# vlazzarini/opencl_fft

Hardware: AMD Instinct MI355X
Metric: Gsamples/s for batched 1D FFT (N=65536, float32) + achieved HBM GB/s vs peak (higher is better)
Workload: dtype f32; 1 GPU; c2c N=65536 x 4096 batches per GPU, float32, in place, device-resident (BASELINE configs[1]); direction=steps alternate forward/inverse plans, kernel=k_fft_res16, global_batch=4096, settle_launches=70, effective_warmup_launches=75, library=opencl_fft_amd/libclfft_amd.so

## Files before the change

include/clfft_amd.h:

```cpp
#ifndef CLFFT_AMD_H
#define CLFFT_AMD_H

#include <stddef.h>

#ifdef __cplusplus
extern "C" {
#endif

#define CLFA_API __attribute__((visibility("default")))

#define CLFA_SUCCESS 0
#define CLFA_DEVICE_NOT_FOUND (-1)
#define CLFA_DEVICE_NOT_AVAILABLE (-2)
#define CLFA_MEM_OBJECT_ALLOCATION_FAILURE (-4)
#define CLFA_OUT_OF_RESOURCES (-5)
#define CLFA_OUT_OF_HOST_MEMORY (-6)
#define CLFA_INVALID_VALUE (-30)
#define CLFA_INVALID_DEVICE (-33)
#define CLFA_INVALID_COMMAND_QUEUE (-36)
#define CLFA_INVALID_MEM_OBJECT (-38)
#define CLFA_INVALID_KERNEL_ARGS (-52)
#define CLFA_INVALID_OPERATION (-59)
#define CLFA_INVALID_BUFFER_SIZE (-61)

// ... 12 lines not shown
CLFA_API int clfa_bitrev_table(int n, int *out);
CLFA_API int clfa_twiddle_table(int n, int forward, float *out);
CLFA_API int clfa_r2c_twiddle_table(int m, int forward, float *out);

CLFA_API int clfa_cfft_create(clfa_fft **plan, int device, int n, int forward);
CLFA_API int clfa_rfft_create(clfa_fft **plan, int device, int size, int forward);
CLFA_API void clfa_fft_destroy(clfa_fft *plan);
CLFA_API int clfa_fft_get_error(const clfa_fft *plan);
CLFA_API const char *clfa_fft_get_log(const clfa_fft *plan);
CLFA_API int clfa_cfft_transform(clfa_fft *plan, float *c, long batch);
CLFA_API int clfa_rfft_transform(clfa_fft *plan, float *c, float *r, long batch);
CLFA_API int clfa_fft_host_alloc(clfa_fft *plan, size_t bytes, void **ptr);
CLFA_API int clfa_fft_host_free(clfa_fft *plan, void *ptr);
CLFA_API int clfa_fft_exec_dev(clfa_fft *plan, void *data, long batch, void *stream);
CLFA_API int clfa_fft_exec_dev_oop(clfa_fft *plan, const void *src, void *dst, long batch, void *stream);
CLFA_API int clfa_fft_device_buffers(clfa_fft *plan, void **data1, void **data2, void **commands);
CLFA_API int clfa_fft_device_tables(clfa_fft *plan, void **w, void **b);
CLFA_API int clfa_copy_to_device(void *stream, void *dst, const void *src, size_t bytes, int blocking);
CLFA_API int clfa_copy_from_device(void *stream, void *dst, const void *src, size_t bytes, int blocking);
CLFA_API int clfa_stream_synchronize(void *stream);
CLFA_API int clfa_fft_run_buffers(clfa_fft *plan);
CLFA_API size_t clfa_fft_workspace_bytes(const clfa_fft *plan);
CLFA_API const char *clfa_fft_kernel_name(const clfa_fft *plan);

CLFA_API int clfa_bandwidth_probe(int device, int what, size_t bytes, int launches, double *tb_per_s);

CLFA_API int clfa_reorder_dev(int device, void *out, const void *in, int n, long batch, void *stream);

CLFA_API int clfa_pconv_create(clfa_pconv **pc, int device, int cvs, int pts, int channels);
CLFA_API void clfa_pconv_destroy(clfa_pconv *pc);
CLFA_API int clfa_pconv_get_error(const clfa_pconv *pc);
CLFA_API int clfa_pconv_nparts(const clfa_pconv *pc);
CLFA_API int clfa_pconv_wp(const clfa_pconv *pc);
CLFA_API int clfa_pconv_wp2(const clfa_pconv *pc);
CLFA_API int clfa_pconv_push_ir(clfa_pconv *pc, const float *ir);
CLFA_API int clfa_pconv_push_ir_dev(clfa_pconv *pc, const void *ir, long channel_stride, void *stream);
CLFA_API int clfa_pconv_convolution(clfa_pconv *pc, float *out, const float *in);
CLFA_API int clfa_pconv_convolution_tv(clfa_pconv *pc, float *out, const float *in1, const float *in2);
CLFA_API int clfa_pconv_process_dev(clfa_pconv *pc, void *out, const void *in1, const void *in2, void *stream);
CLFA_API size_t clfa_pconv_state_bytes(const clfa_pconv *pc);
CLFA_API const char *clfa_pconv_kernel_name(const clfa_pconv *pc);
CLFA_API int clfa_pconv_process_blocks_dev(clfa_pconv *pc, void *out, long out_stride, const void *in1, const void *in2,
                                           long in_stride, long nblocks, void *stream);
CLFA_API int clfa_pconv_convolution_blocks(clfa_pconv *pc, float *out, const float *in1, const float *in2, long nblocks);
CLFA_API size_t clfa_pconv_blocks_workspace_bytes(const clfa_pconv *pc);
CLFA_API const char *clfa_pconv_blocks_kernel_name(const clfa_pconv *pc);
// ... 157 lines not shown
```

opencl_fft_amd/_lib.py:

```python
import ctypes as C
import os

_HERE = os.path.dirname(os.path.abspath(__file__))
LIB_PATH = os.environ.get("CLFA_LIB_PATH") or os.path.join(_HERE, "libclfft_amd.so")
if os.environ.get("CLFA_LIB_PATH"):
    import sys
    print("opencl_fft_amd: CLFA_LIB_PATH is set, loading %s instead of the in-tree library" % LIB_PATH, file=sys.stderr)

_vp, _fp, _ip = C.c_void_p, C.POINTER(C.c_float), C.POINTER(C.c_int)
SYMBOLS = [
    ("clfa_device_count", C.c_int, [_ip]),
    ("clfa_device_name", C.c_int, [C.c_int, C.c_char_p, C.c_size_t]),
    ("clfa_error_string", C.c_char_p, [C.c_int]),
    ("clfa_version", C.c_char_p, []),
    ("clfa_bitrev_table", C.c_int, [C.c_int, _ip]),
    ("clfa_twiddle_table", C.c_int, [C.c_int, C.c_int, _fp]),
    ("clfa_r2c_twiddle_table", C.c_int, [C.c_int, C.c_int, _fp]),
    ("clfa_cfft_create", C.c_int, [C.POINTER(_vp), C.c_int, C.c_int, C.c_int]),
    ("clfa_rfft_create", C.c_int, [C.POINTER(_vp), C.c_int, C.c_int, C.c_int]),
    ("clfa_fft_destroy", None, [_vp]),
    ("clfa_fft_get_error", C.c_int, [_vp]),
    ("clfa_fft_get_log", C.c_char_p, [_vp]),
    ("clfa_cfft_transform", C.c_int, [_vp, _vp, C.c_long]),
    ("clfa_rfft_transform", C.c_int, [_vp, _vp, _vp, C.c_long]),
    ("clfa_fft_host_alloc", C.c_int, [_vp, C.c_size_t, C.POINTER(_vp)]),
    ("clfa_fft_host_free", C.c_int, [_vp, _vp]),
    ("clfa_fft_exec_dev", C.c_int, [_vp, _vp, C.c_long, _vp]),
    ("clfa_fft_exec_dev_oop", C.c_int, [_vp, _vp, _vp, C.c_long, _vp]),
    ("clfa_fft_device_buffers", C.c_int, [_vp, C.POINTER(_vp), C.POINTER(_vp), C.POINTER(_vp)]),
    ("clfa_fft_run_buffers", C.c_int, [_vp]),
    ("clfa_fft_device_tables", C.c_int, [_vp, C.POINTER(_vp), C.POINTER(_vp)]),
    ("clfa_copy_to_device", C.c_int, [_vp, _vp, _vp, C.c_size_t, C.c_int]),
    ("clfa_copy_from_device", C.c_int, [_vp, _vp, _vp, C.c_size_t, C.c_int]),
    ("clfa_stream_synchronize", C.c_int, [_vp]),
    ("clfa_fft_workspace_bytes", C.c_size_t, [_vp]),
    ("clfa_fft_kernel_name", C.c_char_p, [_vp]),
    ("clfa_reorder_dev", C.c_int, [C.c_int, _vp, _vp, C.c_int, C.c_long, _vp]),
    ("clfa_pconv_create", C.c_int, [C.POINTER(_vp), C.c_int, C.c_int, C.c_int, C.c_int]),
    ("clfa_pconv_destroy", None, [_vp]),
    ("clfa_pconv_get_error", C.c_int, [_vp]),
    ("clfa_pconv_nparts", C.c_int, [_vp]),
    ("clfa_pconv_wp", C.c_int, [_vp]),
    ("clfa_pconv_wp2", C.c_int, [_vp]),
    ("clfa_pconv_push_ir", C.c_int, [_vp, _vp]),
    ("clfa_pconv_push_ir_dev", C.c_int, [_vp, _vp, C.c_long, _vp]),
    ("clfa_bandwidth_probe", C.c_int, [C.c_int, C.c_int, C.c_size_t, C.c_int, C.POINTER(C.c_double)]),
    ("clfa_pconv_convolution", C.c_int, [_vp, _vp, _vp]),
    ("clfa_pconv_convolution_tv", C.c_int, [_vp, _vp, _vp, _vp]),
    ("clfa_pconv_process_dev", C.c_int, [_vp, _vp, _vp, _vp, _vp]),
    ("clfa_pconv_state_bytes", C.c_size_t, [_vp]),
    ("clfa_pconv_kernel_name", C.c_char_p, [_vp]),
    ("clfa_pconv_process_blocks_dev", C.c_int, [_vp, _vp, C.c_long, _vp, _vp, C.c_long, C.c_long, _vp]),
    ("clfa_pconv_convolution_blocks", C.c_int, [_vp, _vp, _vp, _vp, C.c_long]),
    ("clfa_pconv_blocks_workspace_bytes", C.c_size_t, [_vp]),
    ("clfa_pconv_blocks_kernel_name", C.c_char_p, [_vp]),
    ("clfa_pconv_matrix_create", C.c_int, [C.POINTER(_vp), C.c_int, C.c_int, C.c_int, C.c_int, C.c_int]),
    ("clfa_pconv_matrix_destroy", None, [_vp]),
    ("clfa_pconv_matrix_get_error", C.c_int, [_vp]),
    ("clfa_pconv_matrix_get_log", C.c_char_p, [_vp]),
# ... 144 lines not shown
```

opencl_fft_amd/csrc/clfft_amd.cpp:

```cpp
#include <utility>

#include "host.hpp"

using namespace clfa;


struct clfa_fft {
  DeviceInfo di;
  FftShape sh;
  int size = 0;
  int err = 0;
  char log[2048];
  hipStream_t stream = nullptr;
  DevBuf half, w2, four, scratch, stage, res16;
  DevBuf own1, own2;
  DevBuf own_w, own_b;
  bool own_tables_ready = false;
  struct Pinned {
    char *h, *d;
    size_t bytes;
  };
  std::vector<Pinned> pinned;
  clfa_fft *own_cplx = nullptr;
  StreamOrder order;
  HostBuf zstage;
  FftTables tabs;
  BigGeom big{};
  DevBuf bigtabs, scratch2;
  clfa_fft *blue_f = nullptr, *blue_i = nullptr;
  DevBuf blue_w, blue_b, blue_work;
};

extern "C" {


const char *clfa_version(void) { return "clfft_amd 0.1 (gfx950)"; }

int clfa_device_count(int *count) {
  if (!count) return CLFA_INVALID_VALUE;
  int c = 0;
  hipError_t e = hipGetDeviceCount(&c);
  if (e != hipSuccess || c <= 0) {
    (void)hipGetLastError();
    *count = 0;
    return CLFA_DEVICE_NOT_FOUND;
  }
  *count = c;
  return CLFA_SUCCESS;
}

int clfa_device_name(int device, char *buf, size_t len) {
// ... 151 lines not shown
    fill_big_tables(h, n, 1 << p->big.logn1);
    if ((e = upload(p->bigtabs, h.data(), sizeof(cpx) * h.size()))) return e;
    const long mb = env_long("CLFA_BIG_CHUNK_MB", 0, 1L << 31);
    const size_t per = sizeof(cpx) * (size_t)n;
    if ((e = p->scratch.ensure(per * chunk_items(per, (size_t)(mb ? mb : 256) << 20)))) return e;
  }
  const unsigned needs = fft_needs(rows);
  auto put = [&](DevBuf &b, const cpx *&tab) {
    const int err = upload(b, h.data(), sizeof(cpx) * h.size());
    tab = (const cpx *)b.p;
    return err;
  };
  if (needs & (kNeedHalf | kNeedHalf2x)) {
    if (needs & kNeedHalf2x) fill_lane_tables(h, rows.logn - 1, rows.logn == 14);
    else if (kLdsTwoLevel(rows.logn)) fill_lane_tables(h, rows.logn, false);
    else fill_twiddle(h, rows.n / 2, rows.n, 1, -1.f);
    if ((e = put(p->half, p->tabs.half))) return e;
  }
  if (needs & kNeedFour) fill_fourstep_tables(h, rows.logn);
  if ((needs & kNeedFour) && (e = put(p->four, p->tabs.four))) return e;
  if (needs & kNeedRes16) fill_res16_tables(h);
  if ((needs & kNeedRes16) && (e = put(p->res16, p->tabs.res16))) return e;
  DevBuf &ws = rows.logn == p->sh.logn ? p->scratch : p->scratch2;
  return needs & kNeedFourWs ? ws.ensure((size_t)fourstep_grid(p->di) * rows.n * sizeof(cpx)) : CLFA_SUCCESS;
}

int clfa_cfft_create(clfa_fft **plan, int device, int n, int forward) {
  return create_object(plan, [&](clfa_fft *p) { return fft_setup(p, device, n, false, n, forward != 0); });
}

int clfa_rfft_create(clfa_fft **plan, int device, int size, int forward) {
  return create_object(plan, [&](clfa_fft *p) {
    if (size < 4 || (size & 1)) {
      snprintf(p->log, sizeof(p->log), "real size must be even, 4..%d (got %d)", 2 << kBigMaxLog, size);
      return CLFA_INVALID_VALUE;
    }
    return fft_setup(p, device, size / 2, true, size, forward != 0);
  });
}

void clfa_fft_destroy(clfa_fft *p) {
  destroy_object(p, [](clfa_fft *q) {
    for (auto &r : q->pinned) (void)hipHostFree(r.h);
    q->pinned.clear();
    if (q->own_cplx) clfa_fft_destroy(q->own_cplx);
    if (q->blue_f) clfa_fft_destroy(q->blue_f);
    if (q->blue_i) clfa_fft_destroy(q->blue_i);
// ... 27 lines not shown
  });
}

static int fft_exec(clfa_fft *p, cpx *d, long off, long batch, hipStream_t s) {
  const FftShape &sh = p->sh;
  const bool fwd = sh.fwd, scale = sh.fwd;
  const FftRoute route = fft_route(sh, batch);
  const bool apart = sh.real && route_pack_apart(route);
  cpx *o = d + off, *scratch = (cpx *)p->scratch.p;
  if (apart && !fwd) {
    HIP_TRY(launch_c2r_unpack(d, p->tabs.w2, sh.n, batch, s, off));
    d = o;
  }
  switch (route) {
    case FftRoute::Lds: HIP_TRY(launch_fft_lds(sh.logn, fwd, fft_mode(sh), scale, d, p->tabs, batch, p->di, s, off)); break;
    case FftRoute::Cfft2x13: HIP_TRY(launch_cfft_2x13(fwd, scale, d, p->tabs, batch, p->di, s, off)); break;
    case FftRoute::Rfft2x13: HIP_TRY(launch_rfft_2x13(fwd, d, p->tabs, batch, p->di, s, off)); break;
    case FftRoute::Rfft2x14: HIP_TRY(launch_rfft_lds15(fwd, d, p->tabs, batch, p->di, s, off)); break;
    case FftRoute::RealRes16:
      if (fwd) HIP_TRY(launch_rfft_res16(d, o, scratch, p->tabs.res16, p->tabs.w2, batch, p->di, s));
      else HIP_TRY(launch_crfft_res16(d, o, scratch, p->tabs.res16, p->tabs.w2, batch, p->di, s));
      break;
    case FftRoute::FourStepSpread:
    case FftRoute::FourStep:
    case FftRoute::Res16: HIP_TRY(launch_fft_4step(sh.logn, fwd, scale, d, scratch, p->tabs, batch, p->di, s, o - d)); break;
    case FftRoute::Big: {
      const int e = for_chunks(batch, (long)(p->scratch.bytes / (sizeof(cpx) * (size_t)sh.n)), [&](long b0, long nb) -> int {
        HIP_TRY(launch_fft_big(p->big, fwd, scale, d + b0 * (long)sh.n, o + b0 * (long)sh.n, scratch, (cpx *)p->scratch2.p,
                               (const cpx *)p->bigtabs.p, p->tabs, nb, p->di, s));
        return CLFA_SUCCESS;
      });
      if (e) return e;
      break;
    }
    case FftRoute::BlueLds:
      HIP_TRY(launch_blue_lds(sh.blue_m, d, o, (const cpx *)p->blue_w.p, (const cpx *)p->blue_b.p, p->blue_f->tabs.half, sh.n,
                              (scale ? 1.0f / (float)sh.n : 1.0f) / (float)sh.blue_m, batch, p->di, s));
      break;
    case FftRoute::Bluestein:
      if (int e = blue_exec(p, d, o, batch, s)) return e;
      break;
  }
  if (apart && fwd) HIP_TRY(launch_r2c_pack(o, p->tabs.w2, sh.n, batch, s));
  return CLFA_SUCCESS;
}

int clfa_fft_exec_dev(clfa_fft *p, void *data, long batch, void *stream) {
  if (int e = obj_error(p)) return e;
  if (!data || batch < 0) return CLFA_INVALID_VALUE;
  if (batch == 0) return CLFA_SUCCESS;
  ENTER_DEVICE(p->di.device);
  hipStream_t s = (hipStream_t)stream;
  HIP_TRY(p->order.use(s));
  return fft_exec(p, (cpx *)data, 0, batch, s);
}

int clfa_fft_exec_dev_oop(clfa_fft *p, const void *src, void *dst, long batch, void *stream) {
  if (int e = obj_error(p)) return e;
  if (!src || !dst || batch < 0) return CLFA_INVALID_VALUE;
  if (src == dst) return clfa_fft_exec_dev(p, dst, batch, stream);
  if (batch == 0) return CLFA_SUCCESS;
  const size_t bytes = sizeof(cpx) * (size_t)p->sh.n * (size_t)batch;
  const char *a = (const char *)src, *b = (const char *)dst;
  if (spans_overlap(a, bytes, b, bytes)) return CLFA_INVALID_VALUE;
  if ((b - a) % (long)sizeof(cpx)) return CLFA_INVALID_VALUE;
  ENTER_DEVICE(p->di.device);
  hipStream_t s = (hipStream_t)stream;
  HIP_TRY(p->order.use(s));
  return fft_exec(p, (cpx *)const_cast<void *>(src), (long)((b - a) / (long)sizeof(cpx)), batch, s);
}

int clfa_fft_device_buffers(clfa_fft *p, void **data1, void **data2, void **commands) {
  if (int e = obj_error(p)) return e;
  ENTER_DEVICE(p->di.device);
  const size_t bytes = sizeof(cpx) * (size_t)p->sh.n;
  int e = p->own1.ensure(bytes);
  if (!e) e = p->own2.ensure(bytes);
  if (e) return e;
  if (data1) *data1 = p->own1.p;
  if (data2) *data2 = p->own2.p;
  if (commands) *commands = (void *)p->stream;
  return CLFA_SUCCESS;
}

int clfa_fft_device_tables(clfa_fft *p, void **w, void **b) {
  if (int e = obj_error(p)) return e;
  if (p->sh.blue_m || p->sh.logn < 1 || p->sh.logn > kMaxLog) return CLFA_INVALID_OPERATION;
  ENTER_DEVICE(p->di.device);
  const int n = p->sh.n;
  if (!p->own_tables_ready) {
    std::vector<cpx> tw;
    fill_twiddle(tw, n, n, 1, p->sh.fwd ? -1.f : 1.f);
// ... 145 lines not shown
```

opencl_fft_amd/csrc/fft_device.hpp:

```cpp
#pragma once
#include <type_traits>

#if defined(__HIPCC__)
#include <hip/hip_runtime.h>
#define CLFA_HD __host__ __device__ __forceinline__
#else
#define CLFA_HD inline
#endif

namespace clfa {

CLFA_HD long xcd_first(unsigned i, unsigned grid) {
  if (grid & 7) return i;
  return (long)(i & 7) * (grid >> 3) + (i >> 3);
}


#if defined(__clang__)
typedef float cpx __attribute__((ext_vector_type(2)));
#define CLFA_VEC 1
#else
struct alignas(8) cpx {
  float x, y;
};
#define CLFA_VEC 0
#endif
#if defined(__HIP_DEVICE_COMPILE__)
#define CLFA_PK 1
#else
#define CLFA_PK 0
#endif

CLFA_HD cpx mk(float x, float y) { cpx r; r.x = x; r.y = y; return r; }
#if CLFA_VEC
CLFA_HD cpx cadd(cpx a, cpx b) { return a + b; }
CLFA_HD cpx csub(cpx a, cpx b) { return a - b; }
CLFA_HD cpx cscale(cpx a, float s) { return a * s; }
#else
// ... 814 lines not shown
```

opencl_fft_amd/csrc/fft_res_blocks.inc:

```

namespace clfa {
namespace {

constexpr int kSpillStride = 400;
constexpr int kXA = 258;
constexpr int kXB = 290;
constexpr int kXSize = 16 * kXB;
constexpr int kTabTw = 0, kTabLo = 256, kTabHi = 512, kTabS = 768, kTabSize = 1792;

__device__ __forceinline__ f4 pack2(cpx a, cpx b) { return f4{a.x, a.y, b.x, b.y}; }

struct HookMap {
  int p[8];
};
constexpr HookMap kMapColA{{0, -1, 1, -1, 2, -1, 3, -1}};
constexpr HookMap kMapColB{{8, -1, 9, -1, 10, -1, 11, -1}};
constexpr HookMap kMapRowC{{0, 1, 2, -1, 3, 4, 5, -1}};
constexpr HookMap kMapRowD{{10, 11, 12, -1, 13, 14, 15, -1}};
struct NoTail {
  __device__ __forceinline__ void operator()() const {}
};
template <bool FWD, class H, int P0, int P1, int P2, int P3, int P4, int P5, int P6, int P7, class T = NoTail>
__device__ __forceinline__ void dft16_hp(cpx (&v)[16], const H &hook, const T &tail = T()) {
  bf4<FWD>(v[0], v[4], v[8], v[12]);
// ... 216 lines not shown
#pragma unroll
    for (int e = 0; e < 16; e++) v[e] = mk(K[RB - kVgprFirst][2 * e], K[RB - kVgprFirst][2 * e + 1]);
  } else {
    acc_fetch<RB - kAgprFirst, INV>(v, std::make_integer_sequence<int, 16>());
  }
}
template <bool FWD, bool LAND = false, bool TWA = true, class H = HookNone>
__device__ __forceinline__ void res_row_block(cpx (&v)[16], const ResLane &L, const H &hook = H()) {
  CLFA_DFT16_H(FWD, v, hook, kMapRowC);
  __syncthreads();
  {
    f4 *pw = reinterpret_cast<f4 *>(L.xb_w);
#pragma unroll
    for (int i = 0; i < 8; i++) pw[i] = pack2(v[2 * i], v[2 * i + 1]);
  }
  __syncthreads();
#pragma unroll
  for (int e = 0; e < 16; e++) v[e] = L.xb_r[18 * e];
  res_tw_rows<FWD, 6, TWA>(v, L, hook);
  if constexpr (LAND) dft16_hp_land<FWD, H, kMapRowD.p[0], kMapRowD.p[1], kMapRowD.p[2], kMapRowD.p[3], kMapRowD.p[4], kMapRowD.p[5], kMapRowD.p[6], kMapRowD.p[7]>(v, hook);
  else CLFA_DFT16_H(FWD, v, hook, kMapRowD);
}

template <bool FWD, int ZC, int NZ, bool LOAD, int N = 16, bool LAST = false>
__device__ __forceinline__ void res_phase1_block(cpx (&v)[16], const ResLane &L, const cpx *x, int cb,
                                                 const int (&so)[16], f32x32 (&K)[kVgprBlk], __amdgpu_buffer_rsrc_t slot,
                                                 const cpx *s_tab, cpx *s_x) {
  res_wait_vm<N>();
  if constexpr (ZC >= 0) acc_fetch_raw<ZC>(v, std::make_integer_sequence<int, 8>());
  else res_land_fetch(v);
  if constexpr (LOAD) {
    const __amdgpu_buffer_rsrc_t r = res_rsrc(x + (cb + 2) * 16);
    if constexpr (NZ >= 0) res_col_block<FWD>(v, L, cb, s_tab, s_x, HookAcc<NZ>{r, L.voff, so});
    else res_col_block<FWD>(v, L, cb, s_tab, s_x, HookLand{r, L.voff, so});
  } else if constexpr (LAST) {
    res_col_block<FWD>(v, L, cb, s_tab, s_x, HookSlot{slot, L.slot_off, so});
  } else {
    res_col_block<FWD>(v, L, cb, s_tab, s_x);
  }
  res_deposit<LAST>(v, L, cb, K, slot);
}

}
}
```

opencl_fft_amd/csrc/fft_res_regs.inc:

```

namespace clfa {
namespace {

#ifndef CLFA_LDNT
#define CLFA_LDNT " nt"
#endif
#ifndef CLFA_STNT
#define CLFA_STNT " nt"
#define CLFA_ST_AUX 2
#endif
typedef unsigned u32x2 __attribute__((ext_vector_type(2)));
typedef float f4 __attribute__((ext_vector_type(4)));
typedef float f32x32 __attribute__((ext_vector_type(32)));

constexpr int kN = 65536;
constexpr int kLdsBlk = 3, kGlbBlk = 1, kVgprBlk = 4, kAgprBlk = 8;
constexpr int kVgprFirst = kLdsBlk + kGlbBlk, kAgprFirst = kVgprFirst + kVgprBlk;
static_assert(kAgprFirst + kAgprBlk == 16, "16 row blocks");

template <int I> __device__ __forceinline__ void acc_write(float v) {
  asm volatile("v_accvgpr_write_b32 a[%0], %1" ::"n"(I), "v"(v));
}
template <int I> __device__ __forceinline__ float acc_read() {
  float v;
// ... 84 lines not shown
__device__ __forceinline__ void res_load_land(const cpx *base, int voff) {
  const __amdgpu_buffer_rsrc_t r = res_rsrc(base);
  res_load_land8<0>(r, voff);
  res_load_land8<8>(r, voff);
}
__device__ __forceinline__ void res_land_fetch(cpx (&v)[16]) {
  asm volatile("v_mov_b64 %0, v[224:225]\n\tv_mov_b64 %1, v[226:227]\n\tv_mov_b64 %2, v[228:229]\n\tv_mov_b64 %3, v[230:231]\n\t"
               "v_mov_b64 %4, v[232:233]\n\tv_mov_b64 %5, v[234:235]\n\tv_mov_b64 %6, v[236:237]\n\tv_mov_b64 %7, v[238:239]"
               : "=v"(v[0]), "=v"(v[1]), "=v"(v[2]), "=v"(v[3]), "=v"(v[4]), "=v"(v[5]), "=v"(v[6]), "=v"(v[7]));
  asm volatile("v_mov_b64 %0, v[240:241]\n\tv_mov_b64 %1, v[242:243]\n\tv_mov_b64 %2, v[244:245]\n\tv_mov_b64 %3, v[246:247]\n\t"
               "v_mov_b64 %4, v[248:249]\n\tv_mov_b64 %5, v[250:251]\n\tv_mov_b64 %6, v[252:253]\n\tv_mov_b64 %7, v[254:255]"
               : "=v"(v[8]), "=v"(v[9]), "=v"(v[10]), "=v"(v[11]), "=v"(v[12]), "=v"(v[13]), "=v"(v[14]), "=v"(v[15]));
}
template <int N> __device__ __forceinline__ void res_wait_vm() {
  static_assert(N == 0 || N == 1 || N == 2 || N == 16 || N == 32 || N == 48, "");
  if constexpr (N == 1) asm volatile("s_waitcnt vmcnt(1)" ::: "memory");
  if constexpr (N == 2) asm volatile("s_waitcnt vmcnt(2)" ::: "memory");
  if constexpr (N == 48) asm volatile("s_waitcnt vmcnt(48)" ::: "memory");
  if constexpr (N == 0) asm volatile("s_waitcnt vmcnt(0)" ::: "memory");
  if constexpr (N == 16) asm volatile("s_waitcnt vmcnt(16)" ::: "memory");
  if constexpr (N == 32) asm volatile("s_waitcnt vmcnt(32)" ::: "memory");
}

template <int K> using ic = std::integral_constant<int, K>;
template <int... I, class F> __device__ __forceinline__ void static_for_(std::integer_sequence<int, I...>, F &&f) { (f(ic<I>()), ...); }
template <int N, class F> __device__ __forceinline__ void static_for(F &&f) { static_for_(std::make_integer_sequence<int, N>(), f); }
struct HookNone {
  template <int K> __device__ __forceinline__ void operator()(ic<K>) const {}
};
template <int CB, bool KEEP = false> struct HookAcc {
  __amdgpu_buffer_rsrc_t r;
  int voff;
  const int (&so)[16];
  template <int K> __device__ __forceinline__ void operator()(ic<K>) const {
    constexpr int lo = 32 * (K & 7) + 2 * (K < 8 ? CB : CB + 1);
#define CLFA_LD_ACC(PRE, POL) \
  asm volatile(PRE "buffer_load_dwordx2 a[%c2:%c3], %0, %1, %4 offen" POL ::"v"(voff), "s"(r), "n"(lo), "n"(lo + 1), "s"(so[K]) : "memory")
    if constexpr (K == 0 && KEEP) CLFA_LD_ACC("s_nop 4\n\t", "");
    else if constexpr (K == 0) CLFA_LD_ACC("s_nop 4\n\t", CLFA_LDNT);
    else if constexpr (KEEP) CLFA_LD_ACC("", "");
    else CLFA_LD_ACC("", CLFA_LDNT);
#undef CLFA_LD_ACC
  }
};
template <bool KEEP = false> struct HookLandT {
  __amdgpu_buffer_rsrc_t r;
// ... 107 lines not shown
```

opencl_fft_amd/csrc/fft_resident.hip:

```cpp
#include <hip/hip_runtime.h>

#include <type_traits>
#include <utility>

#include "internal.hpp"

#include "fft_res_regs.inc"
#include "fft_res_blocks.inc"
#include "fft_res_real.inc"

namespace clfa {
namespace {


template <bool FWD, bool C2R, class LF>
__device__ __forceinline__ void res_phase2_c2c(cpx (&v)[16], const f32x32 (&K)[kVgprBlk], const int (&so)[16], const LF &lane,
                                               const cpx *xn, cpx *y) {
  {
    const ResLane L = lane();
    res_wait_vm<0>();
    res_land_fetch(v);
    res_row_block<FWD, true>(v, L);
  }
  int rb_prev = kLdsBlk;
// ... 83 lines not shown
        const cpx bm = cmul(s_tab[kTabPair + 128], s_tab[kTabPair + 256 + 15 - L.t]);
        res_pair_self_row<false>(v, L.c, L.t, bm, s_c0);
      } else {
        acc_park_flat<kParkAcc>(v);
      }
    }
  }
  {
    const ResLane L = lane(), Lm = lane_m();
    res_store_land(res_rsrc(y + 7 * 16), L.voff, so);
    res_store_so(v, res_rsrc(y + 8 * 16), Lm.voff, so);
    res_load_acc<kZone0>(xn, L.voff);
    res_load_land(xn + 16, L.voff);
  }
}

}

#if defined(__HIP_DEVICE_COMPILE__)
#define CLFA_RES16_TARGET __attribute__((target("no-load-store-opt")))
#else
#define CLFA_RES16_TARGET
#endif
template <bool FWD, bool SCALE, bool R2C = false, bool C2R = false>
__global__ __launch_bounds__(256) __attribute__((amdgpu_num_vgpr(224))) CLFA_RES16_TARGET void k_fft_res16(const cpx *data, cpx *out, cpx *__restrict__ slots,
                                                   const cpx *__restrict__ tabs_g, long batch,
                                                   const cpx *__restrict__ w2_g = nullptr) {
  static_assert(!R2C || (FWD && SCALE && !C2R), "the fused forward pair map");
  static_assert(!C2R || (!FWD && !SCALE), "the fused inverse pair map");
  __shared__ __attribute__((aligned(16))) cpx s_tab[(R2C || C2R) ? kTabSizeR : kTabSize];
  __shared__ __attribute__((aligned(16))) cpx s_x[kXSize];
  __shared__ __attribute__((aligned(16))) char s_spill[256 * kSpillStride];
  __shared__ __attribute__((aligned(16))) cpx s_c0[(R2C || C2R) ? 256 : 1];
  __shared__ __attribute__((aligned(16))) cpx s_col0[C2R ? 2 * kXA : 1];
  acc_claim_all();
  const int tid = threadIdx.x;
  for (int i = tid; i < kTabSize; i += 256) {
    cpx w = tabs_g[i];
    if (SCALE && i >= kTabLo && i < kTabHi) w = cscale(w, R2C ? 0.5f / (float)kN : 1.0f / (float)kN);
    if (C2R && i >= kTabLo && i < kTabHi) w = cscale(w, 0.5f);
    s_tab[i] = w;
  }
  if constexpr (R2C || C2R) {
    s_tab[kTabPair + tid] = w2_g[tid];
    if (tid < 16) s_tab[kTabPair + 256 + tid] = w2_g[256 * tid];
  }
  auto lane = [&]() {
    int l = tid;
    asm volatile("" : "+v"(l));
    ResLane L;
    L.c = l & 15;
    L.t = l >> 4;
// ... 16 lines not shown
    return L;
  };
  [[maybe_unused]] auto lane_b = [&](cpx *save_w, const cpx *save_r) {
    ResLane L = lane();
    const int cm = 16 - L.c, tm = 15 - L.t;
    L.xa_w = (L.c ? s_x + cm * kXA : save_w) + 16 * tm;
    if (L.c == 0) L.xa_r = save_r + L.t;
    return L;
  };
  int so[16];
#pragma unroll
  for (int e = 0; e < 16; e++) {
    so[e] = e * 32768;
    asm volatile("" : "+s"(so[e]));
  }
  const __amdgpu_buffer_rsrc_t slot = res_rsrc(slots + (long)blockIdx.x * 4096);
  __syncthreads();

  f32x32 K[kVgprBlk];
#pragma unroll
  for (int j = 0; j < kVgprBlk; j++) K[j] = 0.f;
  cpx v[16];
  long b = xcd_first(blockIdx.x, gridDim.x);
  if constexpr (C2R) {
    const ResLane L0 = lane();
    const cpx *x0 = data + b * (long)kN;
    res_issue_all(HookAcc<kZone0, kC2rKeepA>{res_rsrc(x0 + 7 * 16), L0.voff, so});
    res_issue_all(HookLandT<true>{res_rsrc(x0 + 8 * 16), (15 - L0.t) * 2048 + (16 - L0.c) * 8, so});
    res_issue_all(HookAcc<kZone1, true>{res_rsrc(x0 + 8 * 16), (15 - L0.t) * 2048 + L0.c * 8, so});
  } else {
    const ResLane L0 = lane();
    res_load_acc<kZone0>(data + b * (long)kN, L0.voff);
    res_load_land(data + b * (long)kN + 16, L0.voff);
  }
#pragma unroll 1
  for (; b < batch; b += gridDim.x) {
    const cpx *x = data + b * (long)kN;
    cpx *y = out + b * (long)kN;
    if constexpr (C2R) {
      res_wait_vm<0>();
      {
        const ResLane L = lane();
        acc_fetch_raw<kZone1>(v, std::make_integer_sequence<int, 8>());
        const cpx bm = cmul(s_tab[kTabPair + 128], s_tab[kTabPair + 256 + 15 - L.t]);
        res_unpair_self_col<false>(v, L.c, L.t, bm, s_c0);
        if (L.c == 0) {
          const HookNone none;
          CLFA_DFT16_H(false, v, none, kMapColA);
          f4 *pw = reinterpret_cast<f4 *>(s_col0 + 16 * (15 - L.t));
#pragma unroll
          for (int i = 0; i < 8; i++) pw[i] = pack2(v[2 * i], v[2 * i + 1]);
        }
      }
      auto pair_step = [&](auto MODE, int p) {
        constexpr int mode = decltype(MODE)::value;
        const int q = 7 - p;
        {
          const ResLane L = lane();
          if (mode == 2) res_wait_vm<kC2rWait ? 1 : 0>();
// ... 20 lines not shown
          res_deposit<false, true>(v, L, q, K, slot);
        }
        {
          const ResLane L = lane_b(s_col0 + ((p + 1) & 1) * kXA, s_col0 + (p & 1) * kXA);
          res_land_fetch(v);
          if constexpr (mode == 0) {
            res_col_block<false>(v, L, 15 - q, s_tab, s_x);
          } else if constexpr (mode == 1) {
            const int voff_m = L.c ? (15 - L.t) * 2048 + (16 - L.c) * 8 : (int)0x80000000;
            res_col_block<false>(v, L, 15 - q, s_tab, s_x, HookLandT<true>{res_rsrc(x + 15 * 16), voff_m, so});
          } else {
            res_col_block<false>(v, L, 15 - q, s_tab, s_x, HookSlot{slot, L.slot_off, so});
          }
          res_deposit<mode == 2, true>(v, L, 15 - q, K, slot);
        }
      };
#pragma unroll 1
      for (int p = 0; p < 6; p++) pair_step(ic<0>(), p);
      pair_step(ic<1>(), 6);
      pair_step(ic<2>(), 7);
    } else {
#pragma unroll 1
      for (int cb = 0; cb < 12; cb += 4) {
        res_phase1_block<FWD, kZone0, kZone1, true>(v, lane(), x, cb, so, K, slot, s_tab, s_x);
        res_phase1_block<FWD, -1, -1, true>(v, lane(), x, cb + 1, so, K, slot, s_tab, s_x);
        res_phase1_block<FWD, kZone1, kZone0, true>(v, lane(), x, cb + 2, so, K, slot, s_tab, s_x);
        res_phase1_block<FWD, -1, -1, true>(v, lane(), x, cb + 3, so, K, slot, s_tab, s_x);
      }
      res_phase1_block<FWD, kZone0, kZone1, true>(v, lane(), x, 12, so, K, slot, s_tab, s_x);
      res_phase1_block<FWD, -1, -1, true>(v, lane(), x, 13, so, K, slot, s_tab, s_x);
      res_phase1_block<FWD, kZone1, -1, false>(v, lane(), x, 14, so, K, slot, s_tab, s_x);
      res_phase1_block<FWD, -1, -1, false, 0, !R2C>(v, lane(), x, 15, so, K, slot, s_tab, s_x);
    }
    long bn = b + gridDim.x;
    bn = bn < batch ? bn : batch - 1;
    const cpx *xn = data + bn * (long)kN;
    if constexpr (R2C) res_phase2_r2c(K, so, slot, lane, lane_m, xn, y, s_tab, s_c0);
    else res_phase2_c2c<FWD, C2R>(v, K, so, lane, xn, y);
  }
}

namespace {

using ResKernel = void (*)(const cpx *, cpx *, cpx *, const cpx *, long, const cpx *);
hipError_t res_launch(ResKernel k, const cpx *data, cpx *out, cpx *slots, const cpx *tabs, const cpx *w2, long batch,
                      const DeviceInfo &di, hipStream_t s) {
  if (batch <= 0) return hipSuccess;
  const int grid = (int)(batch < di.num_cus ? batch : di.num_cus);
  hipLaunchKernelGGL(k, dim3(grid), dim3(256), 0, s, data, out, slots, tabs, batch, w2);
  return hipGetLastError();
}

}

hipError_t launch_fft_res16(bool fwd, bool scale, const cpx *data, cpx *out, cpx *slots, const cpx *tabs, long batch,
                            const DeviceInfo &di, hipStream_t s) {
  if (batch <= 0) return hipSuccess;
  if (!fwd && scale) return hipErrorInvalidValue;
  const ResKernel k = !fwd ? k_fft_res16<false, false> : scale ? k_fft_res16<true, true> : k_fft_res16<true, false>;
  return res_launch(k, data, out, slots, tabs, nullptr, batch, di, s);
}

hipError_t launch_crfft_res16(const cpx *data, cpx *out, cpx *slots, const cpx *tabs, const cpx *w2, long batch,
                              const DeviceInfo &di, hipStream_t s) {
  return res_launch(k_fft_res16<false, false, false, true>, data, out, slots, tabs, w2, batch, di, s);
}

hipError_t launch_rfft_res16(const cpx *data, cpx *out, cpx *slots, const cpx *tabs, const cpx *w2, long batch,
                             const DeviceInfo &di, hipStream_t s) {
  return res_launch(k_fft_res16<true, true, true>, data, out, slots, tabs, w2, batch, di, s);
}

}
```

opencl_fft_amd/csrc/internal.hpp:

```cpp
#pragma once
#include <hip/hip_runtime.h>

#include "fft_device.hpp"
#include "fft_route.hpp"

namespace clfa {

constexpr bool kLdsTwoLevel(int logn) { return logn >= 13; }
constexpr int kLane13Lds = 1280, kLane13Size = 1792;
constexpr int kRow16Stride = kRow16StrideDev;
static_assert(kRow16Stride >= 16 && kRow16Stride % 2 == 0, "rows stay 16-byte aligned");
constexpr int kRow16Lds = 16 * kRow16Stride;
constexpr int kLaneLds = kRow16Lds + (kLane13Lds - 256);
__host__ __device__ constexpr int lane_lds_index(int i) { return i < 256 ? (i >> 4) * kRow16Stride + (i & 15) : i + (kRow16Lds - 256); }
constexpr int kLds14Log = 14, kLane14Size = kLane13Lds + 3 * 1024;

struct FftTables {
  const cpx *half = nullptr;
  const cpx *w2 = nullptr;
  const cpx *four = nullptr;
  const cpx *res16 = nullptr;
};

struct DeviceInfo {
  int device = 0;
  int num_cus = 256;
};

hipError_t launch_fft_lds(int logn, bool fwd, int mode, bool scale, cpx *data, const FftTables &t,
                          long batch, const DeviceInfo &di, hipStream_t s, long out_off = 0);
hipError_t launch_rfft_lds15(bool fwd, cpx *data, const FftTables &t, long batch, const DeviceInfo &di, hipStream_t s,
                             long out_off = 0);
hipError_t launch_rfft_2x13(bool fwd, cpx *data, const FftTables &t, long batch, const DeviceInfo &di, hipStream_t s,
                            long out_off = 0);
hipError_t launch_cfft_2x13(bool fwd, bool scale, cpx *data, const FftTables &t, long batch, const DeviceInfo &di,
                            hipStream_t s, long out_off = 0);

int fourstep_grid(const DeviceInfo &di);
hipError_t launch_fft_4step(int logn, bool fwd, bool scale, cpx *data, cpx *scratch, const FftTables &t, long batch,
                            const DeviceInfo &di, hipStream_t s, long out_off = 0);
int fourstep_split(int logn, int *logn1, int *logn2, int *loglo);
constexpr int kRes16TabSize = 1792;
constexpr size_t kRes16SlotBytes = 32768;
hipError_t launch_fft_res16(bool fwd, bool scale, const cpx *data, cpx *out, cpx *slots, const cpx *tabs, long batch,
                            const DeviceInfo &di, hipStream_t s);
hipError_t launch_rfft_res16(const cpx *data, cpx *out, cpx *slots, const cpx *tabs, const cpx *w2, long batch,
                             const DeviceInfo &di, hipStream_t s);
hipError_t launch_crfft_res16(const cpx *data, cpx *out, cpx *slots, const cpx *tabs, const cpx *w2, long batch,
                              const DeviceInfo &di, hipStream_t s);
constexpr int kBigMaxLog = 24;
struct BigGeom {
  int logn, logn1, logn2;
  bool two_run;
};
int big_split(int logn, BigGeom *g);
hipError_t launch_fft_big(const BigGeom &g, bool fwd, bool scale, cpx *data, cpx *out, cpx *scratch, cpx *scratch2,
                          const cpx *bigtabs, const FftTables &sub, long batch, const DeviceInfo &di, hipStream_t s);

hipError_t launch_r2c_pack(cpx *data, const cpx *w2, int m, long batch, hipStream_t s, long out_off = 0);
hipError_t launch_c2r_unpack(cpx *data, const cpx *w2, int m, long batch, hipStream_t s, long out_off = 0);

constexpr int kBlueMaxN = 1 << 22;
hipError_t launch_blue_lds(int m, const cpx *x, cpx *y, const cpx *w, const cpx *bt, const cpx *tab, int n, float scale,
                           long batch, const DeviceInfo &di, hipStream_t s);
hipError_t launch_blue_pre(const cpx *x, const cpx *w, cpx *a, int n, int m, long batch, hipStream_t s);
hipError_t launch_blue_mul(cpx *a, const cpx *bt, int m, long batch, hipStream_t s);
hipError_t launch_blue_post(const cpx *a, const cpx *w, cpx *x, int n, int m, float scale, long batch, hipStream_t s);

// ... 275 lines not shown
```

opencl_fft_amd/fft.py:

```python
import ctypes as C

import numpy as np

from ._base import CL_INVALID_VALUE, CL_SUCCESS, _Object, _host, _pkg, _ptr_stream
from ._lib import check

PI = 3.141592653589793


def cl_error_string(err):
    return _pkg.lib().clfa_error_string(int(err)).decode()


def device_count():
    n = C.c_int(0)
    _pkg.lib().clfa_device_count(C.byref(n))
    return n.value


def device_name(device=0):
    buf = C.create_string_buffer(256)
    check(_pkg.lib().clfa_device_name(device, buf, 256), "device_name")
    return buf.value.decode()


def bitrev_table(n):
    out = np.empty(n, dtype=np.int32)
    check(_pkg.lib().clfa_bitrev_table(n, out.ctypes.data_as(C.POINTER(C.c_int))), "bitrev_table")
    return out

# ... 28 lines not shown

    def alloc_host(self, shape, dtype):
        dt = np.dtype(dtype)
        n = int(np.prod(shape))
        ptr = C.c_void_p()
        e = _pkg.lib().clfa_fft_host_alloc(self._h, n * dt.itemsize, C.byref(ptr))
        if e != CL_SUCCESS:
            return None
        buf = (C.c_char * (n * dt.itemsize)).from_address(ptr.value)
        return np.frombuffer(buf, dtype=dt, count=n).reshape(shape)

    def free_host(self, array):
        return _pkg.lib().clfa_fft_host_free(self._h, array.ctypes.data)

    def exec_device(self, data, batch, stream=None):
        p, stream = _ptr_stream(data, stream)
        return _pkg.lib().clfa_fft_exec_dev(self._h, p, batch, stream)

    def exec_device_oop(self, src, dst, batch, stream=None):
        ps, stream = _ptr_stream(src, stream)
        pd, _ = _ptr_stream(dst, stream)
        return _pkg.lib().clfa_fft_exec_dev_oop(self._h, ps, pd, batch, stream)


class Clcfft(_Plan):

    def __init__(self, device_id, size, fwd=True):
        self.N = int(size)
        self.forward = bool(fwd)
        self._create(_pkg.lib().clfa_cfft_create, int(device_id), int(size), int(bool(fwd)))

    def transform(self, c):
        c = _host(c, np.complex64)
        if c.shape[-1] != self.N:
            return CL_INVALID_VALUE
        return _pkg.lib().clfa_cfft_transform(self._h, c.ctypes.data, c.size // self.N)


class Clrfft(_Plan):

    def __init__(self, device_id, size, fwd):
        self.size = int(size)
        self.N = self.size // 2
        self.forward = bool(fwd)
        self._create(_pkg.lib().clfa_rfft_create, int(device_id), int(size), int(bool(fwd)))

# ... 24 lines not shown
```

Baseline: 327.4 Gsamples/s.

## Add dynamic per-XCD work stealing to the resident res16 FFT kernel

Replaces the static grid-stride batch assignment in the persistent k_fft_res16 complex kernel with dynamic scheduling. Per-XCD atomic counters let a block claim its next batch from its own XCD's share first, then steal from other XCDs once that share is exhausted. The next batch index is published through shared memory for the prefetch in phase 2. This targets tail imbalance across CUs and XCDs. In exchange it adds atomics, uniform-lane bookkeeping and a counter reset by the last block. It also adds optional per-block balance recording and host APIs to read the counters and records.

```diff
diff --git a/include/clfft_amd.h b/include/clfft_amd.h
--- a/include/clfft_amd.h
+++ b/include/clfft_amd.h
@@ -58,6 +58,9 @@
 CLFA_API int clfa_fft_run_buffers(clfa_fft *plan);
 CLFA_API size_t clfa_fft_workspace_bytes(const clfa_fft *plan);
 CLFA_API const char *clfa_fft_kernel_name(const clfa_fft *plan);
+CLFA_API int clfa_fft_balance_record(clfa_fft *plan, int on);
+CLFA_API int clfa_fft_balance_read(clfa_fft *plan, void *records, int max_records, int *count);
+CLFA_API int clfa_fft_balance_counters(clfa_fft *plan, unsigned *words, int max_words, int *count);
 
 CLFA_API int clfa_bandwidth_probe(int device, int what, size_t bytes, int launches, double *tb_per_s);
 
diff --git a/opencl_fft_amd/_lib.py b/opencl_fft_amd/_lib.py
--- a/opencl_fft_amd/_lib.py
+++ b/opencl_fft_amd/_lib.py
@@ -35,6 +35,9 @@
     ("clfa_stream_synchronize", C.c_int, [_vp]),
     ("clfa_fft_workspace_bytes", C.c_size_t, [_vp]),
     ("clfa_fft_kernel_name", C.c_char_p, [_vp]),
+    ("clfa_fft_balance_record", C.c_int, [_vp, C.c_int]),
+    ("clfa_fft_balance_read", C.c_int, [_vp, _vp, C.c_int, _ip]),
+    ("clfa_fft_balance_counters", C.c_int, [_vp, _vp, C.c_int, _ip]),
     ("clfa_reorder_dev", C.c_int, [C.c_int, _vp, _vp, C.c_int, C.c_long, _vp]),
     ("clfa_pconv_create", C.c_int, [C.POINTER(_vp), C.c_int, C.c_int, C.c_int, C.c_int]),
     ("clfa_pconv_destroy", None, [_vp]),
diff --git a/opencl_fft_amd/csrc/clfft_amd.cpp b/opencl_fft_amd/csrc/clfft_amd.cpp
--- a/opencl_fft_amd/csrc/clfft_amd.cpp
+++ b/opencl_fft_amd/csrc/clfft_amd.cpp
@@ -27,6 +27,10 @@
   FftTables tabs;
   BigGeom big{};
   DevBuf bigtabs, scratch2;
+  unsigned *res16_ctr = nullptr;
+  bool res16_static = false;
+  DevBuf res16_rec;
+  int rec_grid = 0;
   clfa_fft *blue_f = nullptr, *blue_i = nullptr;
   DevBuf blue_w, blue_b, blue_work;
 };
@@ -224,7 +228,19 @@
   if (needs & kNeedRes16) fill_res16_tables(h);
   if ((needs & kNeedRes16) && (e = put(p->res16, p->tabs.res16))) return e;
   DevBuf &ws = rows.logn == p->sh.logn ? p->scratch : p->scratch2;
-  return needs & kNeedFourWs ? ws.ensure((size_t)fourstep_grid(p->di) * rows.n * sizeof(cpx)) : CLFA_SUCCESS;
+  if (!(needs & kNeedFourWs)) return CLFA_SUCCESS;
+  const size_t wsb = (size_t)fourstep_grid(p->di) * rows.n * sizeof(cpx);
+  const bool ctr = !real && (needs & kNeedRes16) && rows.logn == p->sh.logn;
+  if ((e = ws.ensure(wsb + (ctr ? kRes16CtrBytes + 2 * kRes16GuardBytes : 0)))) return e;
+  if (ctr) {
+    char *g = (char *)ws.p + wsb;
+    p->res16_ctr = (unsigned *)(g + kRes16GuardBytes);
+    HIP_TRY(hipMemsetAsync(g, (int)(kRes16GuardWord & 0xff), kRes16CtrBytes + 2 * kRes16GuardBytes, p->stream));
+    HIP_TRY(hipMemsetAsync(p->res16_ctr, 0, kRes16CtrBytes, p->stream));
+    HIP_TRY(hipStreamSynchronize(p->stream));
+    p->res16_static = env_long("CLFA_RES16_STATIC", 0, 2) != 0;
+  }
+  return CLFA_SUCCESS;
 }
 
 int clfa_cfft_create(clfa_fft **plan, int device, int n, int forward) {
@@ -298,8 +314,13 @@
       else HIP_TRY(launch_crfft_res16(d, o, scratch, p->tabs.res16, p->tabs.w2, batch, p->di, s));
       break;
     case FftRoute::FourStepSpread:
-    case FftRoute::FourStep:
-    case FftRoute::Res16: HIP_TRY(launch_fft_4step(sh.logn, fwd, scale, d, scratch, p->tabs, batch, p->di, s, o - d)); break;
+    case FftRoute::FourStep: HIP_TRY(launch_fft_4step(sh.logn, fwd, scale, d, scratch, p->tabs, batch, p->di, s, o - d)); break;
+    case FftRoute::Res16: {
+      ResRecord *rec = (ResRecord *)p->res16_rec.p;
+      if (rec) p->rec_grid = (int)(batch < p->di.num_cus ? batch : p->di.num_cus);
+      HIP_TRY(launch_fft_res16(fwd, scale, d, o, scratch, p->tabs.res16, batch, p->di, s, p->res16_static ? nullptr : p->res16_ctr, rec));
+      break;
+    }
     case FftRoute::Big: {
       const int e = for_chunks(batch, (long)(p->scratch.bytes / (sizeof(cpx) * (size_t)sh.n)), [&](long b0, long nb) -> int {
         HIP_TRY(launch_fft_big(p->big, fwd, scale, d + b0 * (long)sh.n, o + b0 * (long)sh.n, scratch, (cpx *)p->scratch2.p,
@@ -344,6 +365,46 @@
   hipStream_t s = (hipStream_t)stream;
   HIP_TRY(p->order.use(s));
   return fft_exec(p, (cpx *)const_cast<void *>(src), (long)((b - a) / (long)sizeof(cpx)), batch, s);
+}
+
+int clfa_fft_balance_record(clfa_fft *p, int on) {
+  if (int e = obj_error(p)) return e;
+  if (!p->res16_ctr) return CLFA_INVALID_OPERATION;
+  ENTER_DEVICE(p->di.device);
+  HIP_TRY(hipDeviceSynchronize());
+  p->rec_grid = 0;
+  if (!on) {
+    p->res16_rec.release();
+    return CLFA_SUCCESS;
+  }
+  return p->res16_rec.ensure(sizeof(ResRecord) * (size_t)p->di.num_cus);
+}
+
+int clfa_fft_balance_read(clfa_fft *p, void *records, int max_records, int *count) {
+  if (int e = obj_error(p)) return e;
+  if (!records || !count || max_records < 0) return CLFA_INVALID_VALUE;
+  *count = 0;
+  if (!p->res16_rec.p) return CLFA_INVALID_OPERATION;
+  ENTER_DEVICE(p->di.device);
+  HIP_TRY(hipDeviceSynchronize());
+  const int n = p->rec_grid < max_records ? p->rec_grid : max_records;
+  if (n) HIP_TRY(hipMemcpy(records, p->res16_rec.p, sizeof(ResRecord) * (size_t)n, hipMemcpyDeviceToHost));
+  *count = n;
+  return CLFA_SUCCESS;
+}
+
+int clfa_fft_balance_counters(clfa_fft *p, unsigned *words, int max_words, int *count) {
+  if (int e = obj_error(p)) return e;
+  if (!words || !count || max_words < 0) return CLFA_INVALID_VALUE;
+  *count = 0;
+  if (!p->res16_ctr) return CLFA_INVALID_OPERATION;
+  ENTER_DEVICE(p->di.device);
+  HIP_TRY(hipDeviceSynchronize());
+  const int all = (int)((kRes16CtrBytes + 2 * kRes16GuardBytes) / sizeof(unsigned));
+  const int n = all < max_words ? all : max_words;
+  if (n) HIP_TRY(hipMemcpy(words, (const char *)p->res16_ctr - kRes16GuardBytes, sizeof(unsigned) * (size_t)n, hipMemcpyDeviceToHost));
+  *count = n;
+  return CLFA_SUCCESS;
 }
 
 int clfa_fft_device_buffers(clfa_fft *p, void **data1, void **data2, void **commands) {
diff --git a/opencl_fft_amd/csrc/fft_device.hpp b/opencl_fft_amd/csrc/fft_device.hpp
--- a/opencl_fft_amd/csrc/fft_device.hpp
+++ b/opencl_fft_amd/csrc/fft_device.hpp
@@ -14,6 +14,15 @@
   if (grid & 7) return i;
   return (long)(i & 7) * (grid >> 3) + (i >> 3);
 }
+CLFA_HD unsigned xcd_transform(unsigned x, unsigned grid, unsigned p) {
+  const unsigned w = grid >> 3;
+  return (p / w) * grid + x * w + p % w;
+}
+CLFA_HD unsigned xcd_share(unsigned x, unsigned grid, unsigned batch) {
+  const unsigned w = grid >> 3, r = batch % grid, lo = x * w;
+  return (batch / grid) * w + (r <= lo ? 0u : r - lo < w ? r - lo : w);
+}
+CLFA_HD bool xcd_shared_ok(long batch, unsigned grid) { return grid >= 8 && !(grid & 7) && batch > (long)grid && batch < (1L << 31); }
 
 
 #if defined(__clang__)
diff --git a/opencl_fft_amd/csrc/fft_res_blocks.inc b/opencl_fft_amd/csrc/fft_res_blocks.inc
--- a/opencl_fft_amd/csrc/fft_res_blocks.inc
+++ b/opencl_fft_amd/csrc/fft_res_blocks.inc
@@ -262,13 +262,14 @@
   else CLFA_DFT16_H(FWD, v, hook, kMapRowD);
 }
 
-template <bool FWD, int ZC, int NZ, bool LOAD, int N = 16, bool LAST = false>
+template <bool FWD, int ZC, int NZ, bool LOAD, int N = 16, bool LAST = false, class DS = NoTail>
 __device__ __forceinline__ void res_phase1_block(cpx (&v)[16], const ResLane &L, const cpx *x, int cb,
                                                  const int (&so)[16], f32x32 (&K)[kVgprBlk], __amdgpu_buffer_rsrc_t slot,
-                                                 const cpx *s_tab, cpx *s_x) {
+                                                 const cpx *s_tab, cpx *s_x, const DS &draw = DS()) {
   res_wait_vm<N>();
   if constexpr (ZC >= 0) acc_fetch_raw<ZC>(v, std::make_integer_sequence<int, 8>());
   else res_land_fetch(v);
+  draw();
   if constexpr (LOAD) {
     const __amdgpu_buffer_rsrc_t r = res_rsrc(x + (cb + 2) * 16);
     if constexpr (NZ >= 0) res_col_block<FWD>(v, L, cb, s_tab, s_x, HookAcc<NZ>{r, L.voff, so});
diff --git a/opencl_fft_amd/csrc/fft_res_regs.inc b/opencl_fft_amd/csrc/fft_res_regs.inc
--- a/opencl_fft_amd/csrc/fft_res_regs.inc
+++ b/opencl_fft_amd/csrc/fft_res_regs.inc
@@ -130,6 +130,50 @@
   if constexpr (N == 32) asm volatile("s_waitcnt vmcnt(32)" ::: "memory");
 }
 
+template <int REG> __device__ __forceinline__ void res_draw_issue(unsigned *ctr, int byte_off) {
+  asm volatile("v_accvgpr_write_b32 a[%c0], 1\n\ts_nop 4\n\tglobal_atomic_add a[%c0], %1, a[%c0], %2 sc0" ::"n"(REG), "v"(byte_off), "s"(ctr) : "memory");
+}
+constexpr int kDrawStride = 128, kDrawDone = 8;
+__device__ __forceinline__ int res_uniform(int v) { return __builtin_amdgcn_readfirstlane(v); }
+struct ResDraw {
+  int st;
+  int nxt;
+};
+template <int RP, int RC>
+__device__ __forceinline__ void res_draw_step(ResDraw &D, int cb, unsigned *ctr, unsigned grid, unsigned batch, int tid, int *s_next) {
+  asm volatile("" : "+s"(grid), "+s"(batch));
+  const unsigned x = blockIdx.x & 7;
+  int kk = D.st & 15;
+  const int dk = (D.st >> 4) - 1;
+  int pend = -1;
+  if (dk >= 0) {
+    const unsigned d = __builtin_amdgcn_readfirstlane(__builtin_bit_cast(unsigned, acc_read<RP>()));
+    if (dk < kDrawDone) {
+      const unsigned xs = (x + dk) & 7, p = d + (grid >> 3);
+      const bool hit = p < xcd_share(xs, grid, batch);
+      if (hit) D.nxt = res_uniform((int)xcd_transform(xs, grid, p));
+      kk = hit && dk == 0 ? 0 : dk + 1;
+    } else if (d == grid - 1 && tid <= kDrawDone) {
+      unsigned zero = 0;
+      asm volatile("" : "+v"(zero));
+      __hip_atomic_store(ctr + tid * (kDrawStride / 4), zero, __ATOMIC_RELAXED, __HIP_MEMORY_SCOPE_AGENT);
+    }
+  }
+  if (cb < 8) {
+    if (D.nxt < 0 && kk < 8) {
+      if (tid == 0) res_draw_issue<RC>(ctr, (int)(((x + kk) & 7) * kDrawStride));
+      pend = kk;
+    }
+  } else if (cb == 8) {
+    if (tid == 0) *s_next = D.nxt;
+    if (D.nxt < 0) {
+      if (tid == 0) res_draw_issue<RC>(ctr, kDrawDone * kDrawStride);
+      pend = kDrawDone;
+    }
+  }
+  D.st = res_uniform(kk + 16 * (pend + 1));
+}
+
 template <int K> using ic = std::integral_constant<int, K>;
 template <int... I, class F> __device__ __forceinline__ void static_for_(std::integer_sequence<int, I...>, F &&f) { (f(ic<I>()), ...); }
 template <int N, class F> __device__ __forceinline__ void static_for(F &&f) { static_for_(std::make_integer_sequence<int, N>(), f); }
diff --git a/opencl_fft_amd/csrc/fft_resident.hip b/opencl_fft_amd/csrc/fft_resident.hip
--- a/opencl_fft_amd/csrc/fft_resident.hip
+++ b/opencl_fft_amd/csrc/fft_resident.hip
@@ -129,12 +129,23 @@
 #else
 #define CLFA_RES16_TARGET
 #endif
-template <bool FWD, bool SCALE, bool R2C = false, bool C2R = false>
+__device__ __forceinline__ unsigned *res_ctr_of() { return nullptr; }
+__device__ __forceinline__ unsigned *res_ctr_of(unsigned *ctr, ResRecord *) { return ctr; }
+__device__ __forceinline__ ResRecord *res_rec_of() { return nullptr; }
+__device__ __forceinline__ ResRecord *res_rec_of(unsigned *, ResRecord *rec) { return rec; }
+template <bool FWD, bool SCALE, bool R2C = false, bool C2R = false, bool DYN = false, class... X>
 __global__ __launch_bounds__(256) __attribute__((amdgpu_num_vgpr(224))) CLFA_RES16_TARGET void k_fft_res16(const cpx *data, cpx *out, cpx *__restrict__ slots,
                                                    const cpx *__restrict__ tabs_g, long batch,
-                                                   const cpx *__restrict__ w2_g = nullptr) {
+                                                   const cpx *__restrict__ w2_g, X... extra) {
+  static_assert(sizeof...(X) == ((R2C || C2R) ? 0 : 2), "ctr and rec: the complex transforms'");
+  [[maybe_unused]] unsigned *const ctr = res_ctr_of(extra...);
+  [[maybe_unused]] ResRecord *const rec = res_rec_of(extra...);
   static_assert(!R2C || (FWD && SCALE && !C2R), "the fused forward pair map");
   static_assert(!C2R || (!FWD && !SCALE), "the fused inverse pair map");
+  static_assert(!DYN || (!R2C && !C2R), "the packed real transforms keep the static assignment");
+  constexpr bool REC = !R2C && !C2R;
+  [[maybe_unused]] __shared__ int s_next;
+  [[maybe_unused]] unsigned done = 0;
   __shared__ __attribute__((aligned(16))) cpx s_tab[(R2C || C2R) ? kTabSizeR : kTabSize];
   __shared__ __attribute__((aligned(16))) cpx s_x[kXSize];
   __shared__ __attribute__((aligned(16))) char s_spill[256 * kSpillStride];
@@ -197,6 +208,18 @@
   for (int j = 0; j < kVgprBlk; j++) K[j] = 0.f;
   cpx v[16];
   long b = xcd_first(blockIdx.x, gridDim.x);
+  [[maybe_unused]] ResDraw D{0, -1};
+  [[maybe_unused]] auto draw_step = [&](auto RP, auto RC, int cb) {
+    return [&, cb]() {
+      if constexpr (DYN) {
+        int l = tid;
+        asm volatile("" : "+v"(l));
+        if (__builtin_amdgcn_readfirstlane(l) < 64)
+          res_draw_step<decltype(RP)::value, decltype(RC)::value>(D, cb, ctr, gridDim.x, (unsigned)batch, l, &s_next);
+      }
+    };
+  };
+  constexpr int kD0 = 2 * kZone0, kD1 = 2 * kZone0 + 2, kD2 = 2 * kZone1, kD3 = 2 * kZone1 + 2;
   if constexpr (C2R) {
     const ResLane L0 = lane();
     const cpx *x0 = data + b * (long)kN;
@@ -209,7 +232,9 @@
     res_load_land(data + b * (long)kN + 16, L0.voff);
   }
 #pragma unroll 1
-  for (; b < batch; b += gridDim.x) {
+  for (; b < batch;) {
+    if constexpr (REC) done++;
+    if constexpr (DYN) D.nxt = -1;
     const cpx *x = data + b * (long)kN;
     cpx *y = out + b * (long)kN;
     if constexpr (C2R) {
@@ -276,43 +301,73 @@
     } else {
 #pragma unroll 1
       for (int cb = 0; cb < 12; cb += 4) {
+        if constexpr (DYN) {
+          res_phase1_block<FWD, kZone0, kZone1, true, 16, false>(v, lane(), x, cb, so, K, slot, s_tab, s_x, draw_step(ic<kD3>(), ic<kD0>(), cb));
+          res_phase1_block<FWD, -1, -1, true, 16, false>(v, lane(), x, cb + 1, so, K, slot, s_tab, s_x, draw_step(ic<kD0>(), ic<kD1>(), cb + 1));
+          res_phase1_block<FWD, kZone1, kZone0, true, 16, false>(v, lane(), x, cb + 2, so, K, slot, s_tab, s_x, draw_step(ic<kD1>(), ic<kD2>(), cb + 2));
+          res_phase1_block<FWD, -1, -1, true, 16, false>(v, lane(), x, cb + 3, so, K, slot, s_tab, s_x, draw_step(ic<kD2>(), ic<kD3>(), cb + 3));
+        } else {
         res_phase1_block<FWD, kZone0, kZone1, true>(v, lane(), x, cb, so, K, slot, s_tab, s_x);
         res_phase1_block<FWD, -1, -1, true>(v, lane(), x, cb + 1, so, K, slot, s_tab, s_x);
         res_phase1_block<FWD, kZone1, kZone0, true>(v, lane(), x, cb + 2, so, K, slot, s_tab, s_x);
         res_phase1_block<FWD, -1, -1, true>(v, lane(), x, cb + 3, so, K, slot, s_tab, s_x);
+        }
       }
       res_phase1_block<FWD, kZone0, kZone1, true>(v, lane(), x, 12, so, K, slot, s_tab, s_x);
       res_phase1_block<FWD, -1, -1, true>(v, lane(), x, 13, so, K, slot, s_tab, s_x);
       res_phase1_block<FWD, kZone1, -1, false>(v, lane(), x, 14, so, K, slot, s_tab, s_x);
       res_phase1_block<FWD, -1, -1, false, 0, !R2C>(v, lane(), x, 15, so, K, slot, s_tab, s_x);
     }
-    long bn = b + gridDim.x;
-    bn = bn < batch ? bn : batch - 1;
-    const cpx *xn = data + bn * (long)kN;
-    if constexpr (R2C) res_phase2_r2c(K, so, slot, lane, lane_m, xn, y, s_tab, s_c0);
-    else res_phase2_c2c<FWD, C2R>(v, K, so, lane, xn, y);
+    long bn;
+    if constexpr (DYN) {
+      const int nx = __builtin_amdgcn_readfirstlane(s_next);
+      bn = nx < 0 ? b : (long)nx;
+      const cpx *xn = data + bn * (long)kN;
+      res_phase2_c2c<FWD, C2R>(v, K, so, lane, xn, y);
+      b = nx < 0 ? batch : bn;
+    } else {
+      bn = b + gridDim.x;
+      bn = bn < batch ? bn : batch - 1;
+      const cpx *xn = data + bn * (long)kN;
+      if constexpr (R2C) res_phase2_r2c(K, so, slot, lane, lane_m, xn, y, s_tab, s_c0);
+      else res_phase2_c2c<FWD, C2R>(v, K, so, lane, xn, y);
+      b += gridDim.x;
+    }
+  }
+  if constexpr (REC) {
+    if (rec && tid == 0) {
+      rec[blockIdx.x] = ResRecord{done, blockIdx.x & 7, (unsigned long long)wall_clock64()};
+    }
   }
 }
 
 namespace {
 
-using ResKernel = void (*)(const cpx *, cpx *, cpx *, const cpx *, long, const cpx *);
-hipError_t res_launch(ResKernel k, const cpx *data, cpx *out, cpx *slots, const cpx *tabs, const cpx *w2, long batch,
-                      const DeviceInfo &di, hipStream_t s) {
+int res_grid(long batch, const DeviceInfo &di) { return (int)(batch < di.num_cus ? batch : di.num_cus); }
+template <class... X>
+hipError_t res_launch(void (*k)(const cpx *, cpx *, cpx *, const cpx *, long, const cpx *, X...), const cpx *data, cpx *out,
+                      cpx *slots, const cpx *tabs, const cpx *w2, long batch, const DeviceInfo &di, hipStream_t s, X... extra) {
   if (batch <= 0) return hipSuccess;
-  const int grid = (int)(batch < di.num_cus ? batch : di.num_cus);
-  hipLaunchKernelGGL(k, dim3(grid), dim3(256), 0, s, data, out, slots, tabs, batch, w2);
+  hipLaunchKernelGGL(k, dim3(res_grid(batch, di)), dim3(256), 0, s, data, out, slots, tabs, batch, w2, extra...);
   return hipGetLastError();
 }
 
 }
 
 hipError_t launch_fft_res16(bool fwd, bool scale, const cpx *data, cpx *out, cpx *slots, const cpx *tabs, long batch,
-                            const DeviceInfo &di, hipStream_t s) {
+                            const DeviceInfo &di, hipStream_t s, unsigned *ctr, ResRecord *rec) {
   if (batch <= 0) return hipSuccess;
   if (!fwd && scale) return hipErrorInvalidValue;
-  const ResKernel k = !fwd ? k_fft_res16<false, false> : scale ? k_fft_res16<true, true> : k_fft_res16<true, false>;
-  return res_launch(k, data, out, slots, tabs, nullptr, batch, di, s);
+  if (ctr && xcd_shared_ok(batch, (unsigned)res_grid(batch, di))) {
+    const auto k = !fwd ? k_fft_res16<false, false, false, false, true, unsigned *, ResRecord *>
+                   : scale ? k_fft_res16<true, true, false, false, true, unsigned *, ResRecord *>
+                           : k_fft_res16<true, false, false, false, true, unsigned *, ResRecord *>;
+    return res_launch(k, data, out, slots, tabs, (const cpx *)nullptr, batch, di, s, ctr, rec);
+  }
+  const auto k = !fwd ? k_fft_res16<false, false, false, false, false, unsigned *, ResRecord *>
+                 : scale ? k_fft_res16<true, true, false, false, false, unsigned *, ResRecord *>
+                         : k_fft_res16<true, false, false, false, false, unsigned *, ResRecord *>;
+  return res_launch(k, data, out, slots, tabs, (const cpx *)nullptr, batch, di, s, (unsigned *)nullptr, rec);
 }
 
 hipError_t launch_crfft_res16(const cpx *data, cpx *out, cpx *slots, const cpx *tabs, const cpx *w2, long batch,
diff --git a/opencl_fft_amd/csrc/internal.hpp b/opencl_fft_amd/csrc/internal.hpp
--- a/opencl_fft_amd/csrc/internal.hpp
+++ b/opencl_fft_amd/csrc/internal.hpp
@@ -42,8 +42,16 @@
 int fourstep_split(int logn, int *logn1, int *logn2, int *loglo);
 constexpr int kRes16TabSize = 1792;
 constexpr size_t kRes16SlotBytes = 32768;
+constexpr size_t kRes16CtrBytes = 9 * 128;
+constexpr size_t kRes16GuardBytes = 128;
+constexpr unsigned kRes16GuardWord = 0xA5A5A5A5u;
+struct alignas(16) ResRecord {
+  unsigned count;
+  unsigned xcd;
+  unsigned long long stamp;
+};
 hipError_t launch_fft_res16(bool fwd, bool scale, const cpx *data, cpx *out, cpx *slots, const cpx *tabs, long batch,
-                            const DeviceInfo &di, hipStream_t s);
+                            const DeviceInfo &di, hipStream_t s, unsigned *ctr = nullptr, ResRecord *rec = nullptr);
 hipError_t launch_rfft_res16(const cpx *data, cpx *out, cpx *slots, const cpx *tabs, const cpx *w2, long batch,
                              const DeviceInfo &di, hipStream_t s);
 hipError_t launch_crfft_res16(const cpx *data, cpx *out, cpx *slots, const cpx *tabs, const cpx *w2, long batch,
diff --git a/opencl_fft_amd/fft.py b/opencl_fft_amd/fft.py
--- a/opencl_fft_amd/fft.py
+++ b/opencl_fft_amd/fft.py
@@ -6,6 +6,7 @@
 from ._lib import check
 
 PI = 3.141592653589793
+BALANCE_RECORD = np.dtype([("count", np.uint32), ("xcd", np.uint32), ("stamp", np.uint64)])
 
 
 def cl_error_string(err):
@@ -80,6 +81,23 @@
         pd, _ = _ptr_stream(dst, stream)
         return _pkg.lib().clfa_fft_exec_dev_oop(self._h, ps, pd, batch, stream)
 
+    def balance_record(self, on=True):
+        return _pkg.lib().clfa_fft_balance_record(self._h, int(bool(on)))
+
+    def balance_read(self):
+        out = np.zeros(4096, dtype=BALANCE_RECORD)
+        n = C.c_int(0)
+        if _pkg.lib().clfa_fft_balance_read(self._h, out.ctypes.data, len(out), C.byref(n)) != CL_SUCCESS:
+            return None
+        return out[:n.value].copy()
+
+    def balance_counters(self):
+        out = np.zeros(352, dtype=np.uint32)
+        n = C.c_int(0)
+        if _pkg.lib().clfa_fft_balance_counters(self._h, out.ctypes.data, len(out), C.byref(n)) != CL_SUCCESS or n.value != len(out):
+            return None
+        return out[:32].copy(), out[32:320].reshape(9, 32).copy(), out[320:].copy()
+
 
 class Clcfft(_Plan):
 
```

Result: faster. 335.0 Gsamples/s (median of 6 runs) (+2.3%).
